# KaoCC/RayTracing_Simple

Measured on AMD Instinct MI355X. Metric: Mray/s (primary+shadow) at 1080p 64spp, higher is better.
Workload: dtype f32; 1 GPU; C2: Demo scene (6 spheres), 1920x1080, 64 spp, default seed stream; mode=parity, regime=one frame at a time (ms_per_step = ms/frame), kernel=rt_trace_parity_w1, rays_per_frame=177055214, all_rays_per_frame=301710601

## Files before the change

### raytracing_simple_amd/csrc/rt_kernel_fast.hip

```cpp
#define RT_FAST 1
#ifndef RT_DIAGNOSTICS
#define RT_DIAGNOSTICS 0
#endif

#define RT_NS fast
#define RT_KERNEL_NAME rt_trace_fast
#define RT_PACK_KERNEL_NAME rt_pack_fast
#if !RT_DIAGNOSTICS
#define RT_NO_RENDER_KERNEL 1
#endif
#include "rt_trace.inc.h"
#if RT_DIAGNOSTICS
#define RT_SCHED_KERNEL_NAME rt_sched_fast
#include "rt_sched.inc.h"
#endif
#include "rt_opts_reset.h"

#define RT_VARIANT_KERNEL 1

#define RT_NS fast_coop
#define RT_KERNEL_NAME rt_trace_fast_coop
#define RT_OPT_COOP 1
#include "rt_trace.inc.h"
#include "rt_opts_reset.h"

#define RT_NS fast_w1
#define RT_KERNEL_NAME rt_trace_fast_w1
#define RT_OPT_WG_WAVES 1
#define RT_OPT_DIRECT_CAMERA 1
#include "rt_trace.inc.h"
#include "rt_opts_reset.h"

#define RT_NS fast_coop_w1
#define RT_KERNEL_NAME rt_trace_fast_coop_w1
#define RT_OPT_WG_WAVES 1
#define RT_OPT_COOP 1
#include "rt_trace.inc.h"
#include "rt_opts_reset.h"

#define RT_NS fast_pairs
#define RT_KERNEL_NAME rt_trace_fast_pairs
#define RT_OPT_WALK 1
#define RT_OPT_MINWAVES 5
#include "rt_trace.inc.h"
#include "rt_opts_reset.h"

#define RT_NS fast_pairs_g
#define RT_KERNEL_NAME rt_trace_fast_pairs_g
#define RT_OPT_WALK 1
#define RT_OPT_GLOBAL_TABLES 1
#define RT_OPT_MINWAVES 5
#include "rt_trace.inc.h"
#include "rt_opts_reset.h"

#define RT_NS fast_pairs_m
#define RT_KERNEL_NAME rt_trace_fast_pairs_m
#define RT_OPT_WALK 1
#define RT_OPT_GLOBAL_TABLES 2
#define RT_OPT_MINWAVES 5
#include "rt_trace.inc.h"
#include "rt_opts_reset.h"

#define RT_NS fast_g
#define RT_KERNEL_NAME rt_trace_fast_g
#define RT_OPT_GLOBAL_TABLES 1
#include "rt_trace.inc.h"
#include "rt_opts_reset.h"

#if RT_DIAGNOSTICS
#define RT_NS fastdx_w1
#define RT_KERNEL_NAME rt_trace_fastdx_w1
#define RT_OPT_WG_WAVES 1
#define RT_OPT_EXACT_DECISIONS 1
#include "rt_trace.inc.h"
#include "rt_opts_reset.h"

#define RT_NS fastdx_coop_w1
#define RT_KERNEL_NAME rt_trace_fastdx_coop_w1
#define RT_OPT_WG_WAVES 1
#define RT_OPT_COOP 1
#define RT_OPT_EXACT_DECISIONS 1
#include "rt_trace.inc.h"
#include "rt_opts_reset.h"

#define RT_NS fastdx_coop
#define RT_KERNEL_NAME rt_trace_fastdx_coop
#define RT_OPT_COOP 1
#define RT_OPT_EXACT_DECISIONS 1
#include "rt_trace.inc.h"
#include "rt_opts_reset.h"

#define RT_NS fastdx_pairs
#define RT_KERNEL_NAME rt_trace_fastdx_pairs
#define RT_OPT_WALK 1
#define RT_OPT_MINWAVES 5
#define RT_OPT_EXACT_DECISIONS 1
#include "rt_trace.inc.h"
#include "rt_opts_reset.h"

#define RT_NS fast_persist
#define RT_KERNEL_NAME rt_trace_fast_persist
#define RT_OPT_PERSIST 1
#include "rt_trace.inc.h"
#include "rt_opts_reset.h"

#define RT_NS fast_persist_coop
#define RT_KERNEL_NAME rt_trace_fast_persist_coop
#define RT_OPT_PERSIST 1
#define RT_OPT_COOP 1
#include "rt_trace.inc.h"
#include "rt_opts_reset.h"
#endif

namespace rt {

static const Instance kFastInstances[] = {
#if RT_DIAGNOSTICS
    { fast::rt_trace_fast, "rt_trace_fast", 4, kTabSweepLds, kRolePlain, 0 },
#endif
    { fast_w1::rt_trace_fast_w1, "rt_trace_fast_w1", 1, kTabSweepLds, kRolePlain, 0 },
    { fast_coop::rt_trace_fast_coop, "rt_trace_fast_coop", 4, kTabSweepLds, kRoleCoop, kInstStaticCoop },
    { fast_coop_w1::rt_trace_fast_coop_w1, "rt_trace_fast_coop_w1", 1, kTabSweepLds, kRoleCoop, kInstStaticCoop },
    { fast_pairs::rt_trace_fast_pairs, "rt_trace_fast_pairs", 4, kTabPairsLds, kRolePairs, 0 },
    { fast_pairs_g::rt_trace_fast_pairs_g, "rt_trace_fast_pairs_g", 4, kTabPairsGlobal, kRolePairsGlobal, 0 },
    { fast_pairs_m::rt_trace_fast_pairs_m, "rt_trace_fast_pairs_m", 4, kTabPairsLdsSlotsGlobal, kRolePairsMixed, 0 },
    { fast_g::rt_trace_fast_g, "rt_trace_fast_g", 4, kTabSweepGlobal, kRoleSweepGlobal, 0 },
#if RT_DIAGNOSTICS
    { fast::rt_sched_fast, "rt_sched_fast", 4, kTabSweepLds, kRoleNone, kInstNoTileCost },
    { fastdx_w1::rt_trace_fastdx_w1, "rt_trace_fastdx_w1", 1, kTabSweepLds, kRoleNone, 0 },
    { fastdx_coop_w1::rt_trace_fastdx_coop_w1, "rt_trace_fastdx_coop_w1", 1, kTabSweepLds, kRoleNone, kInstStaticCoop },
    { fastdx_coop::rt_trace_fastdx_coop, "rt_trace_fastdx_coop", 4, kTabSweepLds, kRoleNone, kInstStaticCoop },
    { fastdx_pairs::rt_trace_fastdx_pairs, "rt_trace_fastdx_pairs", 4, kTabPairsLds, kRoleNone, 0 },
    { fast_persist::rt_trace_fast_persist, "rt_trace_fast_persist", 4, kTabSweepLds, kRolePersist, kInstPersistent | kInstNoTileCost },
    { fast_persist_coop::rt_trace_fast_persist_coop, "rt_trace_fast_persist_coop", 4, kTabSweepLds, kRolePersistCoop,
      kInstPersistent | kInstNoTileCost | kInstStaticCoop },
#endif
};

const Instance *fast_instances(int *count) {
    *count = (int)(sizeof(kFastInstances) / sizeof(kFastInstances[0]));
    return kFastInstances;
}

hipError_t launch_pack_fast(const LaunchParams &p, hipStream_t stream) {
    if (p.local_rows <= 0 || p.w <= 0) return hipSuccess;
    hipLaunchKernelGGL(fast::rt_pack_fast, dim3((unsigned)((p.w + 63) / 64), (unsigned)((p.local_rows + 3) / 4)),
                       dim3(256), 0, stream, p);
    return hipGetLastError();
}

hipError_t prepare_fast() {
    for (const Instance &k : kFastInstances) {
        hipError_t e = hipFuncSetAttribute(reinterpret_cast<const void *>(k.fn),
                                           hipFuncAttributeMaxDynamicSharedMemorySize, 152 * 1024);
        if (e != hipSuccess) return e;
    }
    return hipSuccess;
}

}
```

### raytracing_simple_amd/csrc/rt_kernel_parity.hip

```cpp
#pragma clang fp contract(off)
#define RT_FAST 0
#ifndef RT_DIAGNOSTICS
#define RT_DIAGNOSTICS 0
#endif

#define RT_NS parity
#define RT_KERNEL_NAME rt_trace_parity
#define RT_PACK_KERNEL_NAME rt_pack_parity
#define RT_OPT_MINWAVES 6
#if !RT_DIAGNOSTICS
#define RT_NO_RENDER_KERNEL 1
#endif
#include "rt_trace.inc.h"
#if RT_DIAGNOSTICS
#undef RT_OPT_MINWAVES
#define RT_OPT_MINWAVES 1
#define RT_SCHED_KERNEL_NAME rt_sched_parity
#include "rt_sched.inc.h"
#endif
#include "rt_opts_reset.h"

#define RT_VARIANT_KERNEL 1

#define RT_NS parity_coop
#define RT_KERNEL_NAME rt_trace_parity_coop
#define RT_OPT_COOP 1
#define RT_OPT_MINWAVES 6
#include "rt_trace.inc.h"
#include "rt_opts_reset.h"

#define RT_NS parity_w1
#define RT_KERNEL_NAME rt_trace_parity_w1
#define RT_OPT_WG_WAVES 1
#define RT_OPT_DIRECT_CAMERA 1
#define RT_OPT_MINWAVES 6
#include "rt_trace.inc.h"
#include "rt_opts_reset.h"

#define RT_NS parity_coop_w1
#define RT_KERNEL_NAME rt_trace_parity_coop_w1
#define RT_OPT_WG_WAVES 1
#define RT_OPT_COOP 1
#define RT_OPT_MINWAVES 6
#include "rt_trace.inc.h"
#include "rt_opts_reset.h"

#define RT_NS parity_pairs
#define RT_KERNEL_NAME rt_trace_parity_pairs
#define RT_WALK_RAYS_KERNEL_NAME rt_walk_rays_parity
#define RT_OPT_WALK 1
#define RT_OPT_MINWAVES 5
#include "rt_trace.inc.h"
#include "rt_opts_reset.h"

#define RT_NS parity_pairs_g
#define RT_KERNEL_NAME rt_trace_parity_pairs_g
#define RT_OPT_WALK 1
#define RT_OPT_GLOBAL_TABLES 1
#define RT_OPT_MINWAVES 5
#include "rt_trace.inc.h"
#include "rt_opts_reset.h"

#define RT_NS parity_pairs_m
#define RT_KERNEL_NAME rt_trace_parity_pairs_m
#define RT_OPT_WALK 1
#define RT_OPT_GLOBAL_TABLES 2
#define RT_OPT_MINWAVES 5
#include "rt_trace.inc.h"
#include "rt_opts_reset.h"

#define RT_NS parity_g
#define RT_KERNEL_NAME rt_trace_parity_g
#define RT_OPT_GLOBAL_TABLES 1
#define RT_OPT_MINWAVES 6
#include "rt_trace.inc.h"
#include "rt_opts_reset.h"

#if RT_DIAGNOSTICS
#define RT_NS parity_pairs_census
#define RT_KERNEL_NAME rt_trace_parity_pairs_census
#define RT_OPT_WALK 2
#include "rt_trace.inc.h"
#include "rt_opts_reset.h"

#define RT_NS parity_pairs_planes
#define RT_KERNEL_NAME rt_trace_parity_pairs_planes
#define RT_OPT_WALK 1
#define RT_OPT_PAIR_PLANES 1
#define RT_OPT_MINWAVES 5
#include "rt_trace.inc.h"
#include "rt_opts_reset.h"

#define RT_NS parity_pairs_2r
#define RT_KERNEL_NAME rt_trace_parity_pairs_2r
#define RT_OPT_WALK 1
#define RT_OPT_RAYS2 1
#define RT_OPT_MINWAVES 3
#include "rt_trace.inc.h"
#include "rt_opts_reset.h"

#define RT_NS parity_pairs_2r_census
#define RT_KERNEL_NAME rt_trace_parity_pairs_2r_census
#define RT_OPT_WALK 2
#define RT_OPT_RAYS2 1
#include "rt_trace.inc.h"
#include "rt_opts_reset.h"

#define RT_NS parity_pairs_g_w4
#define RT_KERNEL_NAME rt_trace_parity_pairs_g_w4
#define RT_OPT_WALK 1
#define RT_OPT_GLOBAL_TABLES 1
#define RT_OPT_MINWAVES 4
#include "rt_trace.inc.h"
#include "rt_opts_reset.h"

#define RT_NS parity_pairs_gt
#define RT_KERNEL_NAME rt_trace_parity_pairs_gt
#define RT_OPT_WALK 1
#define RT_OPT_GLOBAL_TABLES 1
#define RT_OPT_TOP_PAIRS 1
#define RT_OPT_MINWAVES 5
#include "rt_trace.inc.h"
#include "rt_opts_reset.h"

#define RT_NS parity_pairs_gp
#define RT_KERNEL_NAME rt_trace_parity_pairs_gp
#define RT_OPT_WALK 1
#define RT_OPT_GLOBAL_TABLES 1
#define RT_OPT_PREFETCH 1
#define RT_OPT_MINWAVES 5
#include "rt_trace.inc.h"
#include "rt_opts_reset.h"

#define RT_NS parity_pairs_gtp
#define RT_KERNEL_NAME rt_trace_parity_pairs_gtp
#define RT_OPT_WALK 1
#define RT_OPT_GLOBAL_TABLES 1
#define RT_OPT_TOP_PAIRS 1
#define RT_OPT_PREFETCH 1
#define RT_OPT_MINWAVES 5
#include "rt_trace.inc.h"
#include "rt_opts_reset.h"

#define RT_NS parity_pairs_gq
#define RT_KERNEL_NAME rt_trace_parity_pairs_gq
#define RT_OPT_WALK 1
#define RT_OPT_GLOBAL_TABLES 1
#define RT_OPT_PACKED_PAIRS 1
#define RT_OPT_MINWAVES 5
#include "rt_trace.inc.h"
#include "rt_opts_reset.h"

#define RT_NS parity_coop_check
#define RT_KERNEL_NAME rt_trace_parity_coop_check
#define RT_OPT_COOP 2
#include "rt_trace.inc.h"
#include "rt_opts_reset.h"

#define RT_NS parity_census
#define RT_KERNEL_NAME rt_trace_parity_census
#define RT_SCHED_KERNEL_NAME rt_sched_parity_census
#define RT_OPT_STAMPS 1
#include "rt_trace.inc.h"
#include "rt_sched.inc.h"
#include "rt_opts_reset.h"

#define RT_NS parity_coop_census
#define RT_KERNEL_NAME rt_trace_parity_coop_census
#define RT_OPT_COOP 1
#define RT_OPT_STAMPS 1
#include "rt_trace.inc.h"
#include "rt_opts_reset.h"

#define RT_NS parity_persist
#define RT_KERNEL_NAME rt_trace_parity_persist
#define RT_OPT_PERSIST 1
#define RT_OPT_MINWAVES 5
#include "rt_trace.inc.h"
#include "rt_opts_reset.h"

#define RT_NS parity_persist_coop
#define RT_KERNEL_NAME rt_trace_parity_persist_coop
#define RT_OPT_PERSIST 1
#define RT_OPT_COOP 1
#define RT_OPT_MINWAVES 5
#include "rt_trace.inc.h"
#include "rt_opts_reset.h"

#define RT_NS parity_w1_sweptcam
#define RT_KERNEL_NAME rt_trace_parity_w1_sweptcam
#define RT_OPT_WG_WAVES 1
#define RT_OPT_MINWAVES 6
#include "rt_trace.inc.h"
#include "rt_opts_reset.h"

#define RT_NS parity_tl
#define RT_KERNEL_NAME rt_trace_parity_tl
#define RT_OPT_TIMELOG 1
#define RT_OPT_MINWAVES 6
#include "rt_trace.inc.h"
#include "rt_opts_reset.h"
#endif

namespace rt {

static const Instance kParityInstances[] = {
#if RT_DIAGNOSTICS
    { parity::rt_trace_parity, "rt_trace_parity", 4, kTabSweepLds, kRolePlain, 0 },
#endif
    { parity_w1::rt_trace_parity_w1, "rt_trace_parity_w1", 1, kTabSweepLds, kRolePlain, 0 },
    { parity_coop::rt_trace_parity_coop, "rt_trace_parity_coop", 4, kTabSweepLds, kRoleCoop, kInstStaticCoop },
    { parity_coop_w1::rt_trace_parity_coop_w1, "rt_trace_parity_coop_w1", 1, kTabSweepLds, kRoleCoop, kInstStaticCoop },
    { parity_pairs::rt_trace_parity_pairs, "rt_trace_parity_pairs", 4, kTabPairsLds, kRolePairs, 0 },
    { parity_pairs_g::rt_trace_parity_pairs_g, "rt_trace_parity_pairs_g", 4, kTabPairsGlobal, kRolePairsGlobal, 0 },
    { parity_pairs_m::rt_trace_parity_pairs_m, "rt_trace_parity_pairs_m", 4, kTabPairsLdsSlotsGlobal, kRolePairsMixed, 0 },
    { parity_g::rt_trace_parity_g, "rt_trace_parity_g", 4, kTabSweepGlobal, kRoleSweepGlobal, 0 },
#if RT_DIAGNOSTICS
    { parity_pairs_census::rt_trace_parity_pairs_census, "rt_trace_parity_pairs_census", 4, kTabPairsLds, kRoleNone, 0 },
    { parity_pairs_planes::rt_trace_parity_pairs_planes, "rt_trace_parity_pairs_planes", 4, kTabPairsLds, kRoleNone, 0 },
    { parity_pairs_2r::rt_trace_parity_pairs_2r, "rt_trace_parity_pairs_2r", 4, kTabPairsLds, kRoleNone, kInstTwoRays },
    { parity_pairs_2r_census::rt_trace_parity_pairs_2r_census, "rt_trace_parity_pairs_2r_census", 4, kTabPairsLds, kRoleNone, kInstTwoRays },
    { parity_pairs_g_w4::rt_trace_parity_pairs_g_w4, "rt_trace_parity_pairs_g_w4", 4, kTabPairsGlobal, kRoleNone, 0 },
    { parity_pairs_gt::rt_trace_parity_pairs_gt, "rt_trace_parity_pairs_gt", 4, kTabPairsTopLds, kRoleNone, 0 },
    { parity_pairs_gp::rt_trace_parity_pairs_gp, "rt_trace_parity_pairs_gp", 4, kTabPairsGlobal, kRoleNone, 0 },
    { parity_pairs_gq::rt_trace_parity_pairs_gq, "rt_trace_parity_pairs_gq", 4, kTabPairsPacked, kRoleNone, 0 },
    { parity_pairs_gtp::rt_trace_parity_pairs_gtp, "rt_trace_parity_pairs_gtp", 4, kTabPairsTopLds, kRoleNone, 0 },
    { parity_coop_check::rt_trace_parity_coop_check, "rt_trace_parity_coop_check", 4, kTabSweepLds, kRoleNone, kInstStaticCoop },
    { parity_census::rt_trace_parity_census, "rt_trace_parity_census", 4, kTabSweepLds, kRoleNone, 0 },
    { parity_coop_census::rt_trace_parity_coop_census, "rt_trace_parity_coop_census", 4, kTabSweepLds, kRoleNone, kInstStaticCoop },
    { parity::rt_sched_parity, "rt_sched_parity", 4, kTabSweepLds, kRoleNone, kInstNoTileCost },
    { parity_census::rt_sched_parity_census, "rt_sched_parity_census", 4, kTabSweepLds, kRoleNone, kInstNoTileCost },
    { parity_persist::rt_trace_parity_persist, "rt_trace_parity_persist", 4, kTabSweepLds, kRolePersist, kInstPersistent | kInstNoTileCost },
    { parity_persist_coop::rt_trace_parity_persist_coop, "rt_trace_parity_persist_coop", 4, kTabSweepLds, kRolePersistCoop,
      kInstPersistent | kInstNoTileCost | kInstStaticCoop },
    { parity_tl::rt_trace_parity_tl, "rt_trace_parity_tl", 4, kTabSweepLds, kRoleTimelog, 0 },
    { parity_w1_sweptcam::rt_trace_parity_w1_sweptcam, "rt_trace_parity_w1_sweptcam", 1, kTabSweepLds, kRoleNone, 0 },
#endif
};

const Instance *parity_instances(int *count) {
    *count = (int)(sizeof(kParityInstances) / sizeof(kParityInstances[0]));
    return kParityInstances;
}

hipError_t launch_instance(const Instance &inst, const LaunchParams &p, dim3 grid, size_t lds, hipStream_t stream) {
    if (!inst.fn) return hipErrorInvalidValue;
    hipLaunchKernelGGL(inst.fn, grid, dim3(64 * inst.waves), lds, stream, p);
    return hipGetLastError();
}

hipError_t launch_pack_parity(const LaunchParams &p, hipStream_t stream) {
    if (p.local_rows <= 0 || p.w <= 0) return hipSuccess;
    hipLaunchKernelGGL(parity::rt_pack_parity, dim3((unsigned)((p.w + 63) / 64), (unsigned)((p.local_rows + 3) / 4)),
                       dim3(256), 0, stream, p);
    return hipGetLastError();
}

#if RT_DIAGNOSTICS
hipError_t launch_walk_rays(const LaunchParams &p, const float4 *rays, uint32_t n_rays, uint4 *out, size_t lds, hipStream_t stream) {
    if (n_rays == 0) return hipSuccess;
    hipError_t e = hipFuncSetAttribute(reinterpret_cast<const void *>(parity_pairs::rt_walk_rays_parity),
                                       hipFuncAttributeMaxDynamicSharedMemorySize, 152 * 1024);
    if (e != hipSuccess) return e;
    const unsigned blocks = (n_rays + 255) / 256 < 512 ? (n_rays + 255) / 256 : 512;
    hipLaunchKernelGGL(parity_pairs::rt_walk_rays_parity, dim3(blocks), dim3(256), lds, stream, p, rays, n_rays, out);
    return hipGetLastError();
}

hipError_t launch_eval_parity(int op, const float *in, float *out, size_t n, hipStream_t stream) {
    if (n == 0) return hipSuccess;
    hipLaunchKernelGGL(parity::rt_eval_kernel, dim3((unsigned)((n + 255) / 256)), dim3(256), 0,
                       stream, op, in, out, n);
    return hipGetLastError();
}

hipError_t launch_sqrt_check(unsigned long long *d_mismatches, hipStream_t stream, int which) {
    if (which == 1) {
        hipLaunchKernelGGL(parity::rt_hitpost_check_kernel, dim3(256 * 16), dim3(256), 0, stream, d_mismatches);
        return hipGetLastError();
    }
    hipLaunchKernelGGL(parity::rt_sqrt_check_kernel, dim3(256 * 16), dim3(256), 0, stream, d_mismatches);
    return hipGetLastError();
}

hipError_t launch_rcp_probe(unsigned long long *d_hist, hipStream_t stream) {
    hipLaunchKernelGGL(parity::rt_rcp_probe_kernel, dim3(256 * 16), dim3(256), 0, stream, d_hist);
    return hipGetLastError();
}
#endif

hipError_t prepare_parity() {
    for (const Instance &k : kParityInstances) {
        hipError_t e = hipFuncSetAttribute(reinterpret_cast<const void *>(k.fn),
                                           hipFuncAttributeMaxDynamicSharedMemorySize, 152 * 1024);
        if (e != hipSuccess) return e;
    }
    return hipSuccess;
}

}
```

### raytracing_simple_amd/csrc/rt_opts_reset.h

```cpp
#undef RT_NS
#undef RT_KERNEL_NAME
#undef RT_SCHED_KERNEL_NAME
#undef RT_PACK_KERNEL_NAME
#undef RT_WALK_RAYS_KERNEL_NAME
#undef RT_OPT_WG_WAVES
#undef RT_OPT_COOP
#undef RT_OPT_WALK
#undef RT_OPT_GLOBAL_TABLES
#undef RT_OPT_MINWAVES
#undef RT_OPT_PERSIST
#undef RT_OPT_DIRECT_CAMERA
#undef RT_OPT_STAMPS
#undef RT_OPT_TIMELOG
#undef RT_OPT_EXACT_DECISIONS
#undef RT_OPT_PAIR_PLANES
#undef RT_OPT_RAYS2

#undef RT_NO_RENDER_KERNEL
#undef RT_OPT_TOP_PAIRS
#undef RT_OPT_PREFETCH
#undef RT_OPT_PACKED_PAIRS
```

### raytracing_simple_amd/csrc/rt_trace.inc.h

```cpp
#include <hip/hip_runtime.h>

#include "rt_candidates.h"
#include "rt_detmath.h"
#include "rt_device.h"

#ifndef RT_FAST
#error "define RT_FAST to 0 or 1"
#endif
#ifndef RT_DIAGNOSTICS
#define RT_DIAGNOSTICS 0
#endif
#ifndef RT_OPT_WG_WAVES
#define RT_OPT_WG_WAVES 4
#endif
#ifndef RT_OPT_COOP
#define RT_OPT_COOP 0
#endif
#ifndef RT_OPT_WALK
#define RT_OPT_WALK 0
#endif
#ifndef RT_OPT_GLOBAL_TABLES
#define RT_OPT_GLOBAL_TABLES 0
#endif
#ifndef RT_OPT_MINWAVES
#define RT_OPT_MINWAVES 1
#endif
#ifndef RT_OPT_PERSIST
#define RT_OPT_PERSIST 0
#endif
#ifndef RT_OPT_DIRECT_CAMERA
#define RT_OPT_DIRECT_CAMERA 0
#endif
#if RT_OPT_DIRECT_CAMERA && (RT_OPT_GLOBAL_TABLES || RT_OPT_WALK || RT_OPT_PERSIST || RT_OPT_STAMPS)
#error "RT_OPT_DIRECT_CAMERA is for the staged sweep instances only"
#endif
#ifndef RT_OPT_RAYS2
#define RT_OPT_RAYS2 0
#endif
#ifndef RT_OPT_TOP_PAIRS
#define RT_OPT_TOP_PAIRS 0
#endif
#ifndef RT_OPT_PACKED_PAIRS
#define RT_OPT_PACKED_PAIRS 0
#endif
#ifndef RT_OPT_PREFETCH
#define RT_OPT_PREFETCH 0
#endif
#ifndef RT_OPT_PAIR_PLANES
#define RT_OPT_PAIR_PLANES 0
#endif
#ifndef RT_OPT_EXACT_DECISIONS
#define RT_OPT_EXACT_DECISIONS 0
#endif
#ifndef RT_OPT_STAMPS
#define RT_OPT_STAMPS 0
#endif
#ifndef RT_OPT_TIMELOG
#define RT_OPT_TIMELOG 0
#endif


#undef RT_STAMP
#undef RT_STAMP_ROOTS
#if RT_OPT_STAMPS
#define RT_STAMP(k)                                                                          \
    do {                                                                                     \
        asm volatile("; @@SEC " #k);                                                          \
        const unsigned long long b_ = __builtin_amdgcn_ballot_w64(true);                     \
        if ((threadIdx.x & 63) == (unsigned)(__ffsll((long long)b_) - 1))                    \
            atomicAdd(&s_census[k], (1ull << 32) + (unsigned)__popcll(b_));                  \
    } while (0)
#define RT_STAMP_ROOTS(k, cnt)                                                               \
    do {                                                                                     \
        const unsigned long long b_ = __builtin_amdgcn_ballot_w64(true);                     \
        if ((threadIdx.x & 63) == (unsigned)(__ffsll((long long)b_) - 1))                    \
            atomicAdd(&s_census[k], (unsigned long long)(cnt));                              \
    } while (0)
#else
#define RT_STAMP(k)
#define RT_STAMP_ROOTS(k, cnt)
#endif

namespace rt {
namespace RT_NS {

#define RT_EPS 0.01f
#define RT_PI 3.14159265358979323846f

struct V3 {
    float x, y, z;
};

RT_DEV V3 mk(float x, float y, float z) { return V3{ x, y, z }; }
RT_DEV V3 add(V3 a, V3 b) { return mk(a.x + b.x, a.y + b.y, a.z + b.z); }
RT_DEV V3 sub(V3 a, V3 b) { return mk(a.x - b.x, a.y - b.y, a.z - b.z); }
RT_DEV V3 mul(V3 a, V3 b) { return mk(a.x * b.x, a.y * b.y, a.z * b.z); }
RT_DEV V3 scale(V3 a, float k) { return mk(a.x * k, a.y * k, a.z * k); }
RT_DEV float dot(V3 a, V3 b) { return a.x * b.x + a.y * b.y + a.z * b.z; }
RT_DEV float mul_decision(float a, float b) {
    float m = a * b;
#if RT_OPT_EXACT_DECISIONS && RT_FAST
    asm("" : "+v"(m));
#endif
    return m;
}
RT_DEV float dot_decision(V3 a, V3 b) { return mul_decision(a.x, b.x) + mul_decision(a.y, b.y) + mul_decision(a.z, b.z); }
RT_DEV V3 cross(V3 a, V3 b) {
    return mk(a.y * b.z - a.z * b.y, a.z * b.x - a.x * b.z, a.x * b.y - a.y * b.x);
}

RT_DEV float ieee_sqrt_core(float x) {
    float s = __builtin_amdgcn_sqrtf(x);
    const float s_dn = __uint_as_float(__float_as_uint(s) - 1u);
    const float s_up = __uint_as_float(__float_as_uint(s) + 1u);
    const float e_dn = __builtin_fmaf(-s_dn, s, x);
    const float e_up = __builtin_fmaf(-s_up, s, x);
    s = (e_dn <= 0.f) ? s_dn : s;
// ... 152 lines not shown
            if (wave_any_nonneg(p0.det)) { roots += 1; const HitRoots h = hit_roots(p0); if (h.hit && h.t < t) { t = h.t; id = i; } }
            if (wave_any_nonneg(p1.det)) { roots += 1; const HitRoots h = hit_roots(p1); if (h.hit && h.t < t) { t = h.t; id = i + 1; } }
            if (wave_any_nonneg(p2.det)) { roots += 1; const HitRoots h = hit_roots(p2); if (h.hit && h.t < t) { t = h.t; id = i + 2; } }
            if (wave_any_nonneg(p3.det)) { roots += 1; const HitRoots h = hit_roots(p3); if (h.hit && h.t < t) { t = h.t; id = i + 3; } }
            i += 4;
            a = arrived(b);
            if (!more) break;
        }
    }
#endif
    for (; i + 2 <= n; i += 2) {
        const float4 g0 = s_geom[i], g1 = s_geom[i + 1];
        const HitPre p0 = hit_pre(g0, o, d), p1 = hit_pre(g1, o, d);
        if (wave_any_nonneg(p0.det)) {
            roots += 1;
            const HitRoots h0 = hit_roots(p0);
            if (h0.hit && h0.t < t) { t = h0.t; id = i; }
        }
        if (wave_any_nonneg(p1.det)) {
            roots += 1;
            const HitRoots h1 = hit_roots(p1);
            if (h1.hit && h1.t < t) { t = h1.t; id = i + 1; }
        }
    }
    for (; i < n; ++i) {
        const HitPre p0 = hit_pre(s_geom[i], o, d);
        if (wave_any_nonneg(p0.det)) {
            roots += 1;
            const HitRoots h0 = hit_roots(p0);
            if (h0.hit && h0.t < t) { t = h0.t; id = i; }
        }
    }
}

RT_DEV uint32_t sweep_any(const float4 *s_geom, uint32_t n, V3 o, V3 d, float max_t,
                          unsigned long long &roots) {
    uint32_t first = n;
    uint32_t i = 0;
#if RT_OPT_GLOBAL_TABLES && !RT_OPT_WALK
    if (n >= 4) {
        F16 a = arrived(request_four_uniform(s_geom));
        for (;;) {
            const bool more = i + 8 <= n;
            const F16 b = request_four_uniform(s_geom + (more ? i + 4 : i));
            const HitPre p0 = hit_pre(record_of(a, 0), o, d), p1 = hit_pre(record_of(a, 1), o, d), p2 = hit_pre(record_of(a, 2), o, d), p3 = hit_pre(record_of(a, 3), o, d);
            if (__builtin_amdgcn_ballot_w64(first == n && p0.det >= 0.f) != 0ull) { roots += 1; const HitRoots h = hit_roots(p0); if (first == n && h.hit && h.t < max_t) first = i; }
            if (__builtin_amdgcn_ballot_w64(first == n && p1.det >= 0.f) != 0ull) { roots += 1; const HitRoots h = hit_roots(p1); if (first == n && h.hit && h.t < max_t) first = i + 1; }
            if (__builtin_amdgcn_ballot_w64(first == n && p2.det >= 0.f) != 0ull) { roots += 1; const HitRoots h = hit_roots(p2); if (first == n && h.hit && h.t < max_t) first = i + 2; }
            if (__builtin_amdgcn_ballot_w64(first == n && p3.det >= 0.f) != 0ull) { roots += 1; const HitRoots h = hit_roots(p3); if (first == n && h.hit && h.t < max_t) first = i + 3; }
            a = arrived(b);
            if (__builtin_amdgcn_ballot_w64(first == n) == 0ull) return first;
            i += 4;
            if (!more) break;
        }
    }
#endif
    for (; i + 2 <= n; i += 2) {
        const float4 g0 = s_geom[i], g1 = s_geom[i + 1];
        const HitPre p0 = hit_pre(g0, o, d), p1 = hit_pre(g1, o, d);
        if (__builtin_amdgcn_ballot_w64(first == n && p0.det >= 0.f) != 0ull) {
            roots += 1;
            const HitRoots h0 = hit_roots(p0);
            if (first == n && h0.hit && h0.t < max_t) first = i;
        }
        if (__builtin_amdgcn_ballot_w64(first == n && p1.det >= 0.f) != 0ull) {
            roots += 1;
            const HitRoots h1 = hit_roots(p1);
            if (first == n && h1.hit && h1.t < max_t) first = i + 1;
        }
        if (__builtin_amdgcn_ballot_w64(first == n) == 0ull) return first;
    }
    for (; i < n; ++i) {
        const HitPre p0 = hit_pre(s_geom[i], o, d);
        if (__builtin_amdgcn_ballot_w64(first == n && p0.det >= 0.f) != 0ull) {
            roots += 1;
            const HitRoots h0 = hit_roots(p0);
            if (first == n && h0.hit && h0.t < max_t) first = i;
            if (__builtin_amdgcn_ballot_w64(first == n) == 0ull) return first;
        }
    }
    return first;
}

RT_DEV float cos2t_of(float nnt, float ddn) {
#if RT_OPT_EXACT_DECISIONS
    return 1.f - mul_decision(mul_decision(nnt, nnt), 1.f - mul_decision(ddn, ddn));
#else
    return 1.f - nnt * nnt * (1.f - ddn * ddn);
#endif
}
RT_DEV float roulette_p(float Re) {
#if RT_OPT_EXACT_DECISIONS
    return .25f + mul_decision(.5f, Re);
#else
    return .25f + .5f * Re;
#endif
}

RT_DEV bool sample_light(float4 la, float4 lb, uint32_t &s0, uint32_t &s1, uint32_t &c_draws, V3 hp, V3 nl,
                         V3 &sd, float &len, float &numer) {
    float zc = next_random_z(s0, s1);
    float u2 = next_random(s0, s1);
    c_draws += 2;
    float ring = rt_sqrt_unit(fmaxf(0.f, 1.f - zc * zc));
    float sphi, cphi;
#if RT_FAST
    fm_sincos_turns(u2, sphi, cphi);
#else
    dm_sincosf_pos((2.f * RT_PI) * u2, sphi, cphi);
#endif
    V3 us = mk(ring * cphi, ring * sphi, zc);
    V3 on_light = add(scale(us, la.w), mk(la.x, la.y, la.z));
    sd = sub(on_light, hp);
    sd = scale(sd, sqrt_and_rcp(dot(sd, sd), len));
    float wo = dot_decision(sd, us);
    if (wo > 0.f) return false;
    wo = -wo;
    float wi = dot_decision(sd, nl);
    numer = lb.w * wi * wo;
    return wi > 0.f;
}

#if RT_OPT_COOP
constexpr int kCoopSlots = 32;
constexpr int kCoopWaveFloats = kCoopSlots * 9;

RT_DEV uint32_t coop_any(const float4 *s_geom, uint32_t n, bool want, V3 o, V3 d, float max_t, float *scratch, int kmax) {
    const unsigned long long m = __builtin_amdgcn_ballot_w64(want);
    const int K = __popcll(m);
    if (K == 0) return n;
    const unsigned long long present = __builtin_amdgcn_ballot_w64(true);
    const int G = __popcll(present) / K;
    unsigned long long unused_roots = 0;
    if (G < 2 || (kmax > 0 && K > kmax)) {
        uint32_t first = n;
        if (want) first = sweep_any(s_geom, n, o, d, max_t, unused_roots);
        return first;
    }
    float4 *ray_a = reinterpret_cast<float4 *>(scratch);
    float4 *ray_b = ray_a + kCoopSlots;
    uint32_t *res = reinterpret_cast<uint32_t *>(ray_b + kCoopSlots);
    const int rank = __builtin_amdgcn_mbcnt_hi((uint32_t)(m >> 32), __builtin_amdgcn_mbcnt_lo((uint32_t)m, 0u));
    if (want) {
        ray_a[rank] = make_float4(o.x, o.y, o.z, max_t);
        ray_b[rank] = make_float4(d.x, d.y, d.z, 0.f);
        res[rank] = n;
    }
    __builtin_amdgcn_fence(__ATOMIC_RELEASE, "wavefront");
    __builtin_amdgcn_wave_barrier();
    __builtin_amdgcn_fence(__ATOMIC_ACQUIRE, "wavefront");
    const int idx = __builtin_amdgcn_mbcnt_hi((uint32_t)(present >> 32), __builtin_amdgcn_mbcnt_lo((uint32_t)present, 0u));
    const int slot = idx % K;
    const int grp = idx / K;
    if (grp < G) {
        const float4 ra = ray_a[slot];
        const float4 rb = ray_b[slot];
        const V3 ro = mk(ra.x, ra.y, ra.z), rd = mk(rb.x, rb.y, rb.z);
        uint32_t found = n;
        for (uint32_t i = (uint32_t)grp; i < n; i += (uint32_t)G) {
            const HitPre p0 = hit_pre(s_geom[i], ro, rd);
            if (wave_any_nonneg(p0.det)) {
                const HitRoots h0 = hit_roots(p0);
                if (h0.hit && h0.t < ra.w) {
                    found = i;
                    break;
                }
            }
        }
        if (found < n) atomicMin(&res[slot], found);
    }
    __builtin_amdgcn_fence(__ATOMIC_RELEASE, "wavefront");
    __builtin_amdgcn_wave_barrier();
    __builtin_amdgcn_fence(__ATOMIC_ACQUIRE, "wavefront");
    uint32_t first = n;
    if (want) first = res[rank];
    __builtin_amdgcn_wave_barrier();
    return first;
}
#endif


RT_DEV int to_int(float v) {
    float c = fminf(fmaxf(v, 0.f), 1.f);
#if RT_FAST
    float g = fm_powf(c, 1.f / 2.2f);
#else
    float g = dm_powf(c, 1.f / 2.2f);
#endif
    return (int)(g * 255.f + .5f);
}

RT_DEV uint32_t wave_sum(uint32_t v) {
#pragma unroll
    for (int off = 32; off > 0; off >>= 1) v += __shfl_xor(v, off, 64);
    return v;
}

#include "rt_shade.inc.h"

#if RT_OPT_WALK
#include "rt_walk.inc.h"
#elif !defined(RT_NO_RENDER_KERNEL)
extern "C" __global__ void __launch_bounds__(64 * RT_OPT_WG_WAVES, RT_OPT_MINWAVES) RT_KERNEL_NAME(const LaunchParams P) {
// ... 286 lines not shown
                    (const volatile __attribute__((address_space(4))) LaunchParams *)__builtin_amdgcn_kernarg_segment_ptr();
                em4 = mp->scene.emis[id];
                co4 = mp->scene.colr[id];
            }
#else
            if (P.mat_in_lds) {
                em4 = s_emis[id];
                co4 = s_colr[id];
                asm volatile("; materials from LDS" : "+v"(em4.x));
            } else {
                em4 = P.scene.emis[id];
                co4 = P.scene.colr[id];
            }
#endif
            const V3 em = mk(em4.x, em4.y, em4.z);
            col = mk(co4.x, co4.y, co4.z);
            refl = __float_as_int(em4.w);

            hp = add(o, scale(d, t));
            nrm = unit(sub(hp, mk(ge.x, ge.y, ge.z)));
            dp = dot(nrm, d);
            nl = facing_normal(nrm, dp);

            if (!no_emission(em)) {
                if (after_specular) rad = add(rad, emitted(thr, em, dp));
                path_done = true;
            } else if (refl == RT_DIFF) {
                after_specular = false;
                thr = mul(thr, col);
                is_diff = true;
            } else {
                is_gloss = true;
            }
        }

        V3 ld = mk(0.f, 0.f, 0.f);
#if RT_OPT_COOP
        if (__builtin_amdgcn_ballot_w64(is_diff) != 0ull) {
            for (uint32_t j = 0; j < n_lights; ++j) {
                bool want = false;
                V3 sd = mk(0.f, 0.f, 1.f);
                float len = 1.f, numer = 0.f;
                const float4 lb = s_lightB[j];
                if (is_diff) {
                    RT_STAMP(3);
                    want = sample_light(s_lightA[j], lb, s0, s1, c_draws, hp, nl, sd, len, numer);
                }
                RT_STAMP(4);
                const uint32_t first = coop_any(s_geom, n, want, hp, sd, len - RT_EPS, s_coop + wave * kCoopWaveFloats, P.coop_kmax);
#if RT_OPT_COOP == 2
                {
                    unsigned long long dummy = 0;
                    const unsigned long long mm = __builtin_amdgcn_ballot_w64(want);
                    if (want) {
                        const uint32_t ref_first = sweep_any(s_geom, n, hp, sd, len - RT_EPS, dummy);
                        atomicAdd(&P.counters[20], 1ull);
                        if (ref_first != first) {
                            atomicAdd(&P.counters[21], 1ull);
                            P.counters[22] = ((unsigned long long)__popcll(mm) << 48) | ((unsigned long long)first << 24) | ref_first;
                            {
                                const int K_ = __popcll(mm), G_ = 64 / K_;
                                const int rank_ = __builtin_amdgcn_mbcnt_hi((uint32_t)(mm >> 32), __builtin_amdgcn_mbcnt_lo((uint32_t)mm, 0u));
                                const float4 g_ = s_geom[ref_first];
                                const HitPre pp = hit_pre(g_, hp, sd);
                                P.counters[23] = ((unsigned long long)rank_ << 48) | ((unsigned long long)(ref_first % G_) << 32) |
                                                 (unsigned long long)__float_as_uint(pp.det);
                            }
                        }
                    }
                }
#endif
                if (want) {
                    c_shadow += 1;
                    const bool blocked = first < n;
                    c_tests += blocked ? first + 1 : n;
                    if (!blocked) {
                        float k = rt_div(numer, len * len);
                        ld = add(ld, scale(mk(lb.x, lb.y, lb.z), k));
                    }
                }
            }
        }
#else
        if (is_diff) {
            for (uint32_t j = 0; j < n_lights; ++j) {
                RT_STAMP(3);
#if RT_OPT_GLOBAL_TABLES
                const volatile __attribute__((address_space(4))) LaunchParams *lp =
                    (const volatile __attribute__((address_space(4))) LaunchParams *)__builtin_amdgcn_kernarg_segment_ptr();
                const float4 lb = lp->scene.lightB[j];
                const float4 la = lp->scene.lightA[j];
#else
                const float4 lb = s_lightB[j];
                const float4 la = s_lightA[j];
#endif
                V3 sd;
                float len, numer;
                if (!sample_light(la, lb, s0, s1, c_draws, hp, nl, sd, len, numer)) continue;
                c_shadow += 1;
                RT_STAMP(4);
                st_roots_s = 0;
                const uint32_t first = sweep_any(s_geom, n, hp, sd, len - RT_EPS, st_roots_s);
                RT_STAMP_ROOTS(11, st_roots_s);
                const bool blocked = first < n;
                c_tests += blocked ? first + 1 : n;
                if (!blocked) {
                    RT_STAMP(5);
                    float k = rt_div(numer, len * len);
                    ld = add(ld, scale(mk(lb.x, lb.y, lb.z), k));
                }
            }
        }
#endif

        if (is_diff) {
            rad = add(rad, mul(thr, ld));
            RT_STAMP(6);
            float u = next_random(s0, s1);
            float r2 = next_random(s0, s1);
            c_draws += 2;
            float r2s = rt_sqrt_unit(r2);
            const Basis around = basis_around(nl);
            float s1v, c1v;
#if RT_FAST
            fm_sincos_turns(u, s1v, c1v);
#else
            dm_sincosf_pos((2.f * RT_PI) * u, s1v, c1v);
#endif
            V3 nd = cosine_direction(around, s1v, c1v, r2s, r2);
            o = hp;
            d = nd;
        } else if (is_gloss) {
            RT_STAMP(7);
            const float n_dot_d = dp;
            V3 rfl = sub(d, scale(nrm, 2.f * n_dot_d));
            after_specular = true;
            if (refl == RT_SPEC) {
                thr = mul(thr, col);
                d = rfl;
            } else {
                const bool into = dp < 0.f;
                const float ddn = -fabsf(dp);
                const float nc = 1.f, nt = 1.52f;
                float nnt = into ? nc / nt : nt / nc;
                float cos2t = cos2t_of(nnt, ddn);
                if (cos2t < 0.f) {
                    thr = mul(thr, col);
                    d = rfl;
                } else {
                    float kk = (into ? 1.f : -1.f) * (ddn * nnt + rt_sqrt(cos2t));
                    V3 td = unit(sub(scale(d, nnt), scale(nrm, kk)));
                    const float fa = nt - nc, fb = nt + nc;
                    const float R0 = fa * fa / (fb * fb);
                    float c = 1 - (into ? -ddn : dot(td, nrm));
                    float Re = R0 + (1 - R0) * c * c * c * c * c;
                    float Tr = 1.f - Re;
                    float Pr = roulette_p(Re);
                    float pick = next_random(s0, s1);
                    c_draws += 1;
                    const bool take_rfl = pick < Pr;
                    const float wgt = rt_div(take_rfl ? Re : Tr, take_rfl ? Pr : 1.f - Pr);
                    thr = mul(scale(thr, wgt), col);
                    d = take_rfl ? rfl : td;
                }
            }
            o = hp;
        }
        if (is_diff || is_gloss) {
            depth += 1;
            if (depth >= kMaxDepth) path_done = true;
        }

#if RT_OPT_DIRECT_CAMERA
        if (RT_ROTATED) {
            t = 1e20f;
            id = 0;
            if (__builtin_amdgcn_ballot_w64(!path_done) != 0ull) {
                if (!path_done) {
                    sweep_closest(s_geom, n, o, d, t, id, st_roots_c);
                    c_closest += 1;
                }
            }
        } else if (path_done) {
            acc = fold_sample(acc, rad, s, P.first_sample, s_k2, k2_in_lds);
            s += 1;
            need_ray = true;
        }
#else
        if (path_done) {
            RT_STAMP(9);
            acc = fold_sample(acc, rad, s, P.first_sample, s_k2, k2_in_lds);
            s += 1;
            need_ray = true;
        }
#endif
        }
    }

#if !RT_OPT_PERSIST
    KernArgs &Q = *epilogue_args();
    const int lane_e = (int)__builtin_amdgcn_mbcnt_hi(~0u, __builtin_amdgcn_mbcnt_lo(~0u, 0u));
    const bool valid_e = s_end != Q.first_sample;
    if (valid_e && Q.n_samples > 0) {
        const int le = tile_by * kTileH + (lane_e >> 3);
        const XY at = unpack_xy(xy);
        const int xe = at.x, ye = at.y;
        const size_t gid = (size_t)ye * (size_t)Q.w + (size_t)xe;
        const size_t ci = (size_t)(Q.h - ye - 1) * (size_t)Q.w + (size_t)xe;
        float *colors = Q.colors;
        colors[3 * ci] = acc.x;
        colors[3 * ci + 1] = acc.y;
        colors[3 * ci + 2] = acc.z;
        if (!(Q.skip_pixels & 1))
            Q.pixels[(size_t)le * (size_t)Q.w + (size_t)xe] =
                (uint32_t)(to_int(acc.x) | (to_int(acc.y) << 8) | (to_int(acc.z) << 16));
        *reinterpret_cast<uint2 *>(Q.seeds + 2 * gid) = make_uint2(s0, s1);
    }

#endif
#if RT_OPT_PERSIST
    uint32_t n_done = c_samples;
#else
    uint32_t n_done = valid_e ? (uint32_t)Q.n_samples : 0u;
#endif
    uint32_t t_samples = wave_sum(n_done);
    uint32_t t_closest = wave_sum(c_closest);
    uint32_t t_shadow = wave_sum(c_shadow);
    uint32_t t_draws = wave_sum(c_draws);
    unsigned long long tests64 = c_tests + (unsigned long long)c_closest * n;
#pragma unroll
    for (int off = 32; off > 0; off >>= 1) tests64 += __shfl_xor(tests64, off, 64);
#if !RT_OPT_PERSIST
    if (lane_e == 0) atomicMax(&s_tile_cost, (unsigned)(__builtin_amdgcn_s_memrealtime() - s_wg_t0));
    const int lane_c = lane_e;
#else
    const int lane_c = lane;
#endif
    if (lane_c == 0) {
        atomicAdd(&s_stat[0], (unsigned long long)t_samples);
        atomicAdd(&s_stat[1], (unsigned long long)t_closest);
        atomicAdd(&s_stat[2], (unsigned long long)t_shadow);
        atomicAdd(&s_stat[3], tests64);
        atomicAdd(&s_stat[4], (unsigned long long)t_draws);
    }
    __syncthreads();
#if !RT_OPT_PERSIST
    if (tid == 5 && Q.tile_cost) Q.tile_cost[tile_id] = (Q.skip_pixels & 2) ? Q.tile_cost[tile_id] + s_tile_cost : s_tile_cost;
#endif
    if (tid < 5) {
#if RT_OPT_PERSIST
        const unsigned block_linear = blockIdx.x + blockIdx.y * gridDim.x;
#endif
#if RT_OPT_PERSIST
        atomicAdd(&P.stats[(block_linear % (unsigned)kStatReplicas) * 8u + (unsigned)tid], s_stat[tid]);
#else
        atomicAdd(&Q.stats[(block_linear % (unsigned)kStatReplicas) * 8u + (unsigned)tid], s_stat[tid]);
#endif
    }
#if RT_OPT_STAMPS
    __syncthreads();
    if (tid < 12) atomicAdd(&P.counters[8 + tid], s_census[tid]);
#endif
#if RT_OPT_TIMELOG
    {
        const unsigned long long tl_end = __builtin_amdgcn_s_memrealtime();
        if (P.timelog && tid == 0) atomicMax(&P.timelog[8 * (size_t)P.seq + 1], tl_end);
        if (P.wavelog && lane == 0) {
            const size_t wi = ((size_t)(blockIdx.x + blockIdx.y * gridDim.x) * 4 + (size_t)wave) * 3;
            uint32_t hwid, xcc;
            asm volatile("s_getreg_b32 %0, hwreg(HW_REG_HW_ID)" : "=s"(hwid));
            asm volatile("s_getreg_b32 %0, hwreg(HW_REG_XCC_ID)" : "=s"(xcc));
            P.wavelog[wi] = tl_start;
            P.wavelog[wi + 1] = tl_end;
            P.wavelog[wi + 2] = ((unsigned long long)xcc << 32) | hwid;
        }
    }
#endif
}
#undef RT_ROTATED
#endif

#if !defined(RT_VARIANT_KERNEL)
extern "C" __global__ void RT_PACK_KERNEL_NAME(const LaunchParams P) {
    const int x = blockIdx.x * 64 + (threadIdx.x & 63);
    const int lrow = blockIdx.y * 4 + (threadIdx.x >> 6);
    const int tile = lrow / P.tile_rows;
    const int y = (tile * P.nranks + P.rank) * P.tile_rows + (lrow - tile * P.tile_rows);
    if (x >= P.w || lrow >= P.local_rows || y >= P.h) return;
    const size_t ci = (size_t)(P.h - y - 1) * (size_t)P.w + (size_t)x;
    const float r = P.colors[3 * ci], g = P.colors[3 * ci + 1], b = P.colors[3 * ci + 2];
    P.pixels[(size_t)lrow * (size_t)P.w + (size_t)x] = (uint32_t)(to_int(r) | (to_int(g) << 8) | (to_int(b) << 16));
}
#endif

#if !RT_FAST && !defined(RT_VARIANT_KERNEL) && RT_DIAGNOSTICS
extern "C" __global__ void rt_sqrt_check_kernel(unsigned long long *mismatches) {
    const unsigned long long stride = (unsigned long long)gridDim.x * blockDim.x;
    unsigned long long bad = 0;
    for (unsigned long long b = (unsigned long long)blockIdx.x * blockDim.x + threadIdx.x; b < (1ull << 32); b += stride) {
        const float x = __uint_as_float((uint32_t)b);
        const uint32_t a = __float_as_uint(ieee_sqrt_lean(x)), r = __float_as_uint(sqrtf(x));
        const bool both_nan = ((a & 0x7fffffffu) > 0x7f800000u) && ((r & 0x7fffffffu) > 0x7f800000u);
        if (a != r && !both_nan) bad += 1;
    }
    if (bad) atomicAdd(mismatches, bad);
}

extern "C" __global__ void rt_hitpost_check_kernel(unsigned long long *mismatches) {
    const float bs[24] = { 0.f, -0.f, 0x1p-149f, 0x1p-126f, 0x1p-60f, 0x1p-48f, 0x1p-47f, 0x1p-46f, 0x1p-30f,
                           0x1p-24f, 0x1.fffffep-24f, 0x1p-23f, 0x1.000002p-23f, 0x1p-22f, 0.005f, 0x1.47ae12p-7f,
                           0.01f, 0x1.47ae16p-7f, 0.02f, 1.f, 3.f, 1000.f, 1e20f, 3e38f };
    const unsigned long long stride = (unsigned long long)gridDim.x * blockDim.x;
    unsigned long long bad = 0;
    for (unsigned long long k = (unsigned long long)blockIdx.x * blockDim.x + threadIdx.x; k < 0x10000000ull; k += stride) {
        const float det = __uint_as_float((uint32_t)k + 1u);
        for (int j = 0; j < 24; ++j) {
            for (int sg = 0; sg < 2; ++sg) {
                const float b = sg ? -bs[j] : bs[j];
                const float sq_ref = sqrtf(det);
                const float t1r = b - sq_ref, t2r = b + sq_ref;
                const float tr = t1r > RT_EPS ? t1r : (t2r > RT_EPS ? t2r : 0.f);
                const float th = hit_post(HitPre{ b, det });
                const HitRoots hr = hit_roots(HitPre{ b, det });
                if (__float_as_uint(tr) != __float_as_uint(th)) bad += 1;
                if (__float_as_uint(tr) != __float_as_uint(hr.hit ? hr.t : 0.f)) bad += 1;
            }
        }
        uint32_t h1 = (uint32_t)k * 2654435761u + 0x9e3779b9u, h2 = ((uint32_t)k ^ 0x85ebca6bu) * 2246822519u;
        h1 ^= h1 >> 15; h1 *= 2246822519u; h1 ^= h1 >> 13;
        h2 ^= h2 >> 16; h2 *= 3266489917u; h2 ^= h2 >> 14;
        const float rb = __uint_as_float(h1), rdet = __uint_as_float(h2);
        const float sq = sqrtf(rdet);
        const float t1 = rb - sq, t2 = rb + sq;
        float tr = t1 > RT_EPS ? t1 : (t2 > RT_EPS ? t2 : 0.f);
        tr = rdet < 0.f ? 0.f : tr;
        const HitRoots hr = hit_roots(HitPre{ rb, rdet });
        if (__float_as_uint(tr) != __float_as_uint(hr.hit ? hr.t : 0.f)) bad += 1;
    }
    if (bad) atomicAdd(mismatches, bad);
// ... 48 lines not shown
```

Before: 75600 Mray/s.

## Fuse last light's shadow test with next-bounce closest-hit sweep sharing origin terms

In the rotated direct-camera w1 loop, the shadow ray for the last light is deferred and traced in the same sphere sweep as the next bounce's closest-hit ray. Both rays start at the same hit point, so the origin-to-center vector and its squared length are computed once per sphere for both tests. The aim is to remove one full pass over the geometry table and the repeated per-sphere setup arithmetic. The cost is more complex control flow, extra live registers, and reordered random draws that must still match parity. The old behaviour is kept as new twosweeps instances, and the epilogue's stats indexing is changed to use the lane index.

```diff
diff --git a/raytracing_simple_amd/csrc/rt_kernel_fast.hip b/raytracing_simple_amd/csrc/rt_kernel_fast.hip
--- a/raytracing_simple_amd/csrc/rt_kernel_fast.hip
+++ b/raytracing_simple_amd/csrc/rt_kernel_fast.hip
@@ -28,6 +28,7 @@
 #define RT_KERNEL_NAME rt_trace_fast_w1
 #define RT_OPT_WG_WAVES 1
 #define RT_OPT_DIRECT_CAMERA 1
+#define RT_OPT_SHARED_ORIGIN 1
 #include "rt_trace.inc.h"
 #include "rt_opts_reset.h"
 
@@ -98,6 +99,13 @@
 #include "rt_trace.inc.h"
 #include "rt_opts_reset.h"
 
+#define RT_NS fast_w1_twosweeps
+#define RT_KERNEL_NAME rt_trace_fast_w1_twosweeps
+#define RT_OPT_WG_WAVES 1
+#define RT_OPT_DIRECT_CAMERA 1
+#include "rt_trace.inc.h"
+#include "rt_opts_reset.h"
+
 #define RT_NS fast_persist
 #define RT_KERNEL_NAME rt_trace_fast_persist
 #define RT_OPT_PERSIST 1
@@ -131,6 +139,7 @@
     { fastdx_coop_w1::rt_trace_fastdx_coop_w1, "rt_trace_fastdx_coop_w1", 1, kTabSweepLds, kRoleNone, kInstStaticCoop },
     { fastdx_coop::rt_trace_fastdx_coop, "rt_trace_fastdx_coop", 4, kTabSweepLds, kRoleNone, kInstStaticCoop },
     { fastdx_pairs::rt_trace_fastdx_pairs, "rt_trace_fastdx_pairs", 4, kTabPairsLds, kRoleNone, 0 },
+    { fast_w1_twosweeps::rt_trace_fast_w1_twosweeps, "rt_trace_fast_w1_twosweeps", 1, kTabSweepLds, kRoleNone, 0 },
     { fast_persist::rt_trace_fast_persist, "rt_trace_fast_persist", 4, kTabSweepLds, kRolePersist, kInstPersistent | kInstNoTileCost },
     { fast_persist_coop::rt_trace_fast_persist_coop, "rt_trace_fast_persist_coop", 4, kTabSweepLds, kRolePersistCoop,
       kInstPersistent | kInstNoTileCost | kInstStaticCoop },
diff --git a/raytracing_simple_amd/csrc/rt_kernel_parity.hip b/raytracing_simple_amd/csrc/rt_kernel_parity.hip
--- a/raytracing_simple_amd/csrc/rt_kernel_parity.hip
+++ b/raytracing_simple_amd/csrc/rt_kernel_parity.hip
@@ -33,6 +33,7 @@
 #define RT_KERNEL_NAME rt_trace_parity_w1
 #define RT_OPT_WG_WAVES 1
 #define RT_OPT_DIRECT_CAMERA 1
+#define RT_OPT_SHARED_ORIGIN 1
 #define RT_OPT_MINWAVES 6
 #include "rt_trace.inc.h"
 #include "rt_opts_reset.h"
@@ -190,6 +191,14 @@
 #define RT_NS parity_w1_sweptcam
 #define RT_KERNEL_NAME rt_trace_parity_w1_sweptcam
 #define RT_OPT_WG_WAVES 1
+#define RT_OPT_MINWAVES 6
+#include "rt_trace.inc.h"
+#include "rt_opts_reset.h"
+
+#define RT_NS parity_w1_twosweeps
+#define RT_KERNEL_NAME rt_trace_parity_w1_twosweeps
+#define RT_OPT_WG_WAVES 1
+#define RT_OPT_DIRECT_CAMERA 1
 #define RT_OPT_MINWAVES 6
 #include "rt_trace.inc.h"
 #include "rt_opts_reset.h"
@@ -235,6 +244,7 @@
       kInstPersistent | kInstNoTileCost | kInstStaticCoop },
     { parity_tl::rt_trace_parity_tl, "rt_trace_parity_tl", 4, kTabSweepLds, kRoleTimelog, 0 },
     { parity_w1_sweptcam::rt_trace_parity_w1_sweptcam, "rt_trace_parity_w1_sweptcam", 1, kTabSweepLds, kRoleNone, 0 },
+    { parity_w1_twosweeps::rt_trace_parity_w1_twosweeps, "rt_trace_parity_w1_twosweeps", 1, kTabSweepLds, kRoleNone, 0 },
 #endif
 };
 
diff --git a/raytracing_simple_amd/csrc/rt_opts_reset.h b/raytracing_simple_amd/csrc/rt_opts_reset.h
--- a/raytracing_simple_amd/csrc/rt_opts_reset.h
+++ b/raytracing_simple_amd/csrc/rt_opts_reset.h
@@ -10,6 +10,7 @@
 #undef RT_OPT_MINWAVES
 #undef RT_OPT_PERSIST
 #undef RT_OPT_DIRECT_CAMERA
+#undef RT_OPT_SHARED_ORIGIN
 #undef RT_OPT_STAMPS
 #undef RT_OPT_TIMELOG
 #undef RT_OPT_EXACT_DECISIONS
diff --git a/raytracing_simple_amd/csrc/rt_trace.inc.h b/raytracing_simple_amd/csrc/rt_trace.inc.h
--- a/raytracing_simple_amd/csrc/rt_trace.inc.h
+++ b/raytracing_simple_amd/csrc/rt_trace.inc.h
@@ -33,6 +33,12 @@
 #endif
 #if RT_OPT_DIRECT_CAMERA && (RT_OPT_GLOBAL_TABLES || RT_OPT_WALK || RT_OPT_PERSIST || RT_OPT_STAMPS)
 #error "RT_OPT_DIRECT_CAMERA is for the staged sweep instances only"
+#endif
+#ifndef RT_OPT_SHARED_ORIGIN
+#define RT_OPT_SHARED_ORIGIN 0
+#endif
+#if RT_OPT_SHARED_ORIGIN && (!RT_OPT_DIRECT_CAMERA || RT_OPT_COOP)
+#error "RT_OPT_SHARED_ORIGIN is for the rotated loop of the plain sweep instances"
 #endif
 #ifndef RT_OPT_RAYS2
 #define RT_OPT_RAYS2 0
@@ -351,6 +357,61 @@
     return first;
 }
 
+#if RT_OPT_SHARED_ORIGIN
+struct OriginPre {
+    V3 op;
+    float oo;
+};
+RT_DEV OriginPre origin_pre(float4 g, V3 o) {
+    const V3 op = mk(g.x - o.x, g.y - o.y, g.z - o.z);
+#if RT_OPT_EXACT_DECISIONS
+    return OriginPre{ op, dot_decision(op, op) };
+#else
+    return OriginPre{ op, dot(op, op) };
+#endif
+}
+RT_DEV HitPre hit_pre_from(OriginPre q, float r2, V3 d) {
+#if RT_OPT_EXACT_DECISIONS
+    const float b = dot_decision(q.op, d);
+    return HitPre{ b, mul_decision(b, b) - q.oo + r2 };
+#else
+    const float b = dot(q.op, d);
+    return HitPre{ b, b * b - q.oo + r2 };
+#endif
+}
+struct BothPre {
+    HitPre ps, pc;
+};
+RT_DEV BothPre both_pre(float4 g, V3 o, V3 sd, V3 d) {
+    const OriginPre q = origin_pre(g, o);
+    return BothPre{ hit_pre_from(q, g.w, sd), hit_pre_from(q, g.w, d) };
+}
+RT_DEV void both_roots(BothPre p, uint32_t i, uint32_t n, uint32_t &first, float max_t, unsigned long long go_mask, float &t, uint32_t &id) {
+    const HitPre ps = p.ps, pc = p.pc;
+    if (__builtin_amdgcn_ballot_w64(first == n && ps.det >= 0.f) != 0ull) {
+        const HitRoots h = hit_roots(ps);
+        if (first == n && h.hit && h.t < max_t) first = i;
+    }
+    if ((__builtin_amdgcn_ballot_w64(pc.det >= 0.f) & go_mask) != 0ull) {
+        const HitRoots h = hit_roots(pc);
+        if (h.hit && h.t < t) { t = h.t; id = i; }
+    }
+}
+RT_DEV void sweep_both(const float4 *s_geom, uint32_t n, V3 o, uint32_t &first, V3 sd, float max_t, bool go, V3 d, float &t, uint32_t &id) {
+    const unsigned long long go_mask = __builtin_amdgcn_ballot_w64(go);
+    if (!go) t = 0.f;
+    uint32_t i = 0;
+    for (; i + 2 <= n; i += 2) {
+        const float4 g0 = s_geom[i], g1 = s_geom[i + 1];
+        const BothPre p0 = both_pre(g0, o, sd, d), p1 = both_pre(g1, o, sd, d);
+        both_roots(p0, i, n, first, max_t, go_mask, t, id);
+        both_roots(p1, i + 1, n, first, max_t, go_mask, t, id);
+    }
+    for (; i < n; ++i) both_roots(both_pre(s_geom[i], o, sd, d), i, n, first, max_t, go_mask, t, id);
+    if (t == 0.f) t = 1e20f;
+}
+#endif
+
 RT_DEV float cos2t_of(float nnt, float ddn) {
 #if RT_OPT_EXACT_DECISIONS
     return 1.f - mul_decision(mul_decision(nnt, nnt), 1.f - mul_decision(ddn, ddn));
@@ -366,11 +427,7 @@
 #endif
 }
 
-RT_DEV bool sample_light(float4 la, float4 lb, uint32_t &s0, uint32_t &s1, uint32_t &c_draws, V3 hp, V3 nl,
-                         V3 &sd, float &len, float &numer) {
-    float zc = next_random_z(s0, s1);
-    float u2 = next_random(s0, s1);
-    c_draws += 2;
+RT_DEV bool sample_light_drawn(float4 la, float4 lb, float zc, float u2, V3 hp, V3 nl, V3 &sd, float &len, float &numer) {
     float ring = rt_sqrt_unit(fmaxf(0.f, 1.f - zc * zc));
     float sphi, cphi;
 #if RT_FAST
@@ -388,6 +445,13 @@
     float wi = dot_decision(sd, nl);
     numer = lb.w * wi * wo;
     return wi > 0.f;
+}
+RT_DEV bool sample_light(float4 la, float4 lb, uint32_t &s0, uint32_t &s1, uint32_t &c_draws, V3 hp, V3 nl,
+                         V3 &sd, float &len, float &numer) {
+    float zc = next_random_z(s0, s1);
+    float u2 = next_random(s0, s1);
+    c_draws += 2;
+    return sample_light_drawn(la, lb, zc, u2, hp, nl, sd, len, numer);
 }
 
 #if RT_OPT_COOP
@@ -840,8 +904,14 @@
             }
         }
 #else
+#if RT_OPT_SHARED_ORIGIN
+        const uint32_t n_swept = (RT_ROTATED && n_lights != 0u) ? n_lights - 1u : n_lights;
+        float kept_zc = 0.f, kept_u2 = 0.f;
+#else
+        const uint32_t n_swept = n_lights;
+#endif
         if (is_diff) {
-            for (uint32_t j = 0; j < n_lights; ++j) {
+            for (uint32_t j = 0; j < n_swept; ++j) {
                 RT_STAMP(3);
 #if RT_OPT_GLOBAL_TABLES
                 const volatile __attribute__((address_space(4))) LaunchParams *lp =
@@ -868,10 +938,20 @@
                     ld = add(ld, scale(mk(lb.x, lb.y, lb.z), k));
                 }
             }
+#if RT_OPT_SHARED_ORIGIN
+            if (n_swept != n_lights) {
+                kept_zc = next_random_z(s0, s1);
+                kept_u2 = next_random(s0, s1);
+                c_draws += 2;
+            }
+#endif
         }
 #endif
 
         if (is_diff) {
+#if RT_OPT_SHARED_ORIGIN
+            if (!RT_ROTATED)
+#endif
             rad = add(rad, mul(thr, ld));
             RT_STAMP(6);
             float u = next_random(s0, s1);
@@ -933,12 +1013,45 @@
         if (RT_ROTATED) {
             t = 1e20f;
             id = 0;
+#if RT_OPT_SHARED_ORIGIN
+            uint32_t first = is_diff ? n + 1u : n + 2u;
+            V3 sd = mk(0.f, 0.f, 1.f);
+            float max_t = 0.f, k = 0.f;
+            if (is_diff && n_swept != n_lights) {
+                float len, numer;
+                if (sample_light_drawn(s_lightA[n_swept], s_lightB[n_swept], kept_zc, kept_u2, o, nl, sd, len, numer)) {
+                    c_shadow += 1;
+                    first = n;
+                    max_t = len - RT_EPS;
+                    k = rt_div(numer, len * len);
+                }
+            }
+            if (__builtin_amdgcn_ballot_w64(first == n) != 0ull) {
+                if (!path_done) c_closest += 1;
+                sweep_both(s_geom, n, o, first, sd, max_t, !path_done, d, t, id);
+            } else if (__builtin_amdgcn_ballot_w64(!path_done) != 0ull) {
+                if (!path_done) {
+                    sweep_closest(s_geom, n, o, d, t, id, st_roots_c);
+                    c_closest += 1;
+                }
+            }
+            if (first <= n) {
+                const bool blocked = first < n;
+                c_tests += blocked ? first + 1 : n;
+                if (!blocked) {
+                    const float4 lb = s_lightB[n_swept];
+                    ld = add(ld, scale(mk(lb.x, lb.y, lb.z), k));
+                }
+            }
+            if (first != n + 2u) rad = add(rad, mul(thr, ld));
+#else
             if (__builtin_amdgcn_ballot_w64(!path_done) != 0ull) {
                 if (!path_done) {
                     sweep_closest(s_geom, n, o, d, t, id, st_roots_c);
                     c_closest += 1;
                 }
             }
+#endif
         } else if (path_done) {
             acc = fold_sample(acc, rad, s, P.first_sample, s_k2, k2_in_lds);
             s += 1;
@@ -1002,17 +1115,22 @@
         atomicAdd(&s_stat[4], (unsigned long long)t_draws);
     }
     __syncthreads();
+#if RT_OPT_SHARED_ORIGIN && RT_OPT_WG_WAVES == 1
+    const int tid_e = lane_e;
+#else
+    const int tid_e = tid;
+#endif
 #if !RT_OPT_PERSIST
-    if (tid == 5 && Q.tile_cost) Q.tile_cost[tile_id] = (Q.skip_pixels & 2) ? Q.tile_cost[tile_id] + s_tile_cost : s_tile_cost;
-#endif
-    if (tid < 5) {
+    if (tid_e == 5 && Q.tile_cost) Q.tile_cost[tile_id] = (Q.skip_pixels & 2) ? Q.tile_cost[tile_id] + s_tile_cost : s_tile_cost;
+#endif
+    if (tid_e < 5) {
 #if RT_OPT_PERSIST
         const unsigned block_linear = blockIdx.x + blockIdx.y * gridDim.x;
 #endif
 #if RT_OPT_PERSIST
-        atomicAdd(&P.stats[(block_linear % (unsigned)kStatReplicas) * 8u + (unsigned)tid], s_stat[tid]);
-#else
-        atomicAdd(&Q.stats[(block_linear % (unsigned)kStatReplicas) * 8u + (unsigned)tid], s_stat[tid]);
+        atomicAdd(&P.stats[(block_linear % (unsigned)kStatReplicas) * 8u + (unsigned)tid_e], s_stat[tid_e]);
+#else
+        atomicAdd(&Q.stats[(block_linear % (unsigned)kStatReplicas) * 8u + (unsigned)tid_e], s_stat[tid_e]);
 #endif
     }
 #if RT_OPT_STAMPS
```

New measurement: 78900 Mray/s, median of 6. 1.04x the previous value.
